# NoakLiu/FastFourierDiffusion

Measured on AMD Instinct MI355X. Metric: samples/sec at 1000 diffusion steps, ECG freq-domain, higher is better.
Workload: dtype f32; 1 GPU; ECG frequency-domain L=187 C=1, transformer d72/H12/NL10/F2048, VP beta[0.1,20], 1000-step sampler (BASELINE configs[1]); batch_per_gpu=512, global_batch=512, diffusion_steps=1000, cache=False, noise=philox on device

## Files before the change

### fastfourierdiffusion_amd/csrc/ffd_api.hip

```cpp
#include <math.h>
#include <stdarg.h>
#include <stdio.h>
#include <string.h>

#include <algorithm>
#include <string>
#include <vector>

#include "../../include/ffd.h"
#include "ffd_internal.h"

using namespace ffd;

namespace {

template <typename T>
struct Grow {
  T* p = nullptr;
  size_t cap = 0;
};

struct WeightSlot {
  std::string key;
  size_t n;
// ... 204 lines not shown
  if (g_ffn_split) {
    p.ffn = FFN_SPLIT;
  } else if (hp && g_ffn_height == 1) {
    p.ffn = FFN_LN_OPROJ, p.mb = hp;
  } else if (!(hp && g_small_wgs == 0) && (p.ns = small_path_splits(M, d, F))) {
    p.ffn = FFN_SMALL, p.part_floats = small_path_partial_floats(M, d, p.ns);
  } else if (pk.ring && !(hp && g_rows_slices == 0) && rows_slice_plan(M, d, F, &p.nw, &p.nslice, &unf)) {
    p.ffn = unf ? FFN_ROWS_SLICED : FFN_ROWS_SLICED_OPROJ, p.cps = 2, p.part_floats = rows_slice_floats(M, d, p.nslice);
  } else if ((p.nm = hp && g_mid_path == 1 ? 0 : mid_path_splits(M, d, F))) {
    p.ffn = FFN_MID, p.part_floats = small_path_partial_floats(cdiv(M, 64) * 64, d, p.nm);
  } else if (pk.ring && ffn_rows_fused_selected(M, d, F)) {
    p.ffn = FFN_ROWS_OPROJ, p.nw = rows_nw(), p.cps = 2;
  } else if (pk.ring && ffn_rows_selected(M, d, F)) {
    p.ffn = FFN_ROWS, p.nw = rows_nw(), p.cps = g_ffn_rows_cps == 1 && d == 72 ? 1 : 2;
  } else {
    p.ffn = FFN_LN;
    p.mb = g_ffn_mb_override >= 1 ? g_ffn_mb_override : cdiv(M, 64) >= 512 ? 4 : cdiv(M, 32) >= 512 ? 2 : 1;
    if (hp) p.mb = hp;
    p.persist = g_ffn_persist;
  }
  if (p.ffn == FFN_LN || p.ffn == FFN_LN_OPROJ) p.rem = g_ffn_rem && ffn_rem_rows(d, p.mb);
  p.oproj_separate = p.ffn >= FFN_ROWS_SLICED;
  p.swap = p.ffn == FFN_ROWS_SLICED_OPROJ || p.ffn == FFN_ROWS_OPROJ;
  return p;
}

LstmPlan plan_lstm(const ffd_model_desc& m, int B) {
  const int maxb = lstm_wave_max_batch(m.max_len, m.d_model);
  if (g_lstm_wave && m.d_model % 4 == 0 && m.d_model >= 16 && m.num_layers <= 64 && maxb >= 16)
    return {true, B < maxb ? B : maxb};
  return {false, B};
}

}

extern "C" {

int ffd_tune(const char* key, int value) {
  if (!key) return FFD_ERR_INVALID;
  if (!strcmp(key, "reset")) {
#define FFD_KNOB_RESET(k, var, def, ...) var = def;
    FFD_KNOBS(FFD_KNOB_RESET, FFD_KNOB_RESET)
#undef FFD_KNOB_RESET
    return FFD_OK;
  }
  const int v = value;
// ... 387 lines not shown
                                hipStream_t s, unsigned long long* stamp = nullptr) {
  const ffd_model_desc& m = ctx->desc;
  const int L = m.max_len, d = m.d_model, H = m.n_head, hd = d / H;
  float* out = ctx->attn.p;
  if (p.attn == ATTN_FUSED) {
    const float* pack = p.q_only == 2 ? w.aw_kvq
                        : p.hpw == 2  ? (p.q_only ? w.aw_q2 : w.aw_full2)
                                      : (p.q_only ? w.aw_q : w.aw_full);
    return launch_qkv_attention(AttnArgs{x, pack, kt, vt, kt_out, vt_out, out, B, L, n_own, stamp,
                                         p.attn_static && w.attn_bounded && kt == nullptr},
                                d, hd, p.hpw, p.q_only, p.kspl, p.qg, s);
  }
  if (stamp != nullptr) return hipErrorInvalidValue;
  const size_t M = (size_t)B * L;
  float *q = ctx->qkv.p, *k = q + M * d, *v = q + 2 * M * d;
  hipError_t e = launch_linear_hm(x, p.q_only ? w.q_wp : w.in_wp, w.in_b, q, k, v, (int)M, p.q_only ? 1 : 3, d, L, H, hd, s);
  if (e == hipSuccess) e = launch_attention(q, k, v, kt, vt, out, B, L, H, hd, n_own, p.qg, s);
  if (e == hipSuccess && kt_out)
    e = launch_kv_store(k, v, kt_out, vt_out, L, H, hd, n_own, s);
  return e;
}

static hipError_t run_ffn(const ffd_ctx* ctx, const LayerPlan& p, const LayerWeights& w, const float* attn, float* cur,
                          float* alt, int M, hipStream_t s, unsigned long long* stamp = nullptr) {
  const int d = ctx->desc.d_model, F = ctx->desc.dim_feedforward;
  float* P = ctx->ffn_part.p;
  const bool sliced = p.ffn == FFN_ROWS_SLICED_OPROJ || p.ffn == FFN_ROWS_SLICED;
  const bool fused = p.ffn == FFN_ROWS_SLICED_OPROJ || p.ffn == FFN_ROWS_OPROJ;
  float* const y = fused ? alt : cur;
  const RowsArgs rows{fused ? attn : alt, fused ? cur : nullptr, &w, sliced ? P : y, M, d, F, p.nw, p.cps, fused,
                      sliced ? p.nslice : 0, stamp};
  switch (p.ffn) {
    case FFN_LN_OPROJ:
      return stamp ? hipErrorInvalidValue : launch_oproj_ffn_ln(attn, cur, w, cur, M, d, F, p.mb, p.rem, s);
    case FFN_SMALL:
      return stamp ? hipErrorInvalidValue : launch_oproj_ffn_small(attn, cur, w, alt, P, cur, M, d, F, p.ns, s);
    case FFN_ROWS_SLICED_OPROJ:
    case FFN_ROWS_SLICED: {
      if (stamp || p.nslice < 2) return hipErrorInvalidValue;
      const hipError_t e = launch_ffn_rows(rows, s);
      return e != hipSuccess ? e : launch_rows_reduce_ln(P, w, y, M, d, p.nslice, s);
    }
    case FFN_ROWS_OPROJ:
    case FFN_ROWS: return launch_ffn_rows(rows, s);
    case FFN_MID:
      return stamp ? hipErrorInvalidValue : launch_ffn_mid(alt, w, P, cur, M, d, F, p.nm, s);
    case FFN_SPLIT: return launch_ffn_ln_split(alt, w, cur, M, d, F, s, stamp);
    case FFN_LN: return launch_ffn_ln(alt, w, cur, M, d, F, p.mb, p.rem, p.persist, s, stamp);
  }
  return hipErrorInvalidValue;
}

static const struct {
  const char* name;
  bool oproj;
} kFfnForms[] = {
    {"k_ffn_ln<oproj>", true},
    {"k_oproj_ffn_split + k_ffn_reduce_ln", true},
    {"k_ffn_rows<oproj, sliced> + k_rows_reduce_ln", true},
    {"k_ffn_rows<oproj>", true},
    {"k_ffn_rows<sliced> + k_rows_reduce_ln", false},
    {"k_ffn_part", false},
    {"k_ffn_ln_split", false},
    {"k_ffn_rows", false},
    {"k_ffn_ln", false},
};

static int forward_impl(ffd_ctx* ctx, const float* x, const float* temb, int temb_stride, float* score_out,
                        float* crf_out, int B, int n_rec, hipStream_t s, const float** hidden_out = nullptr) {
  const ffd_model_desc& m = ctx->desc;
  const int L = m.max_len, C = m.n_channels, d = m.d_model, M = B * L;
  const ModelWeights& mw = ctx->model;
  if (m.kind == FFD_MODEL_MLP) {
    const int io = L * C, F = m.dim_feedforward;
    HIPCHECK(launch_dense(x, mw.embed_w, mw.embed_b, temb_stride ? nullptr : temb, temb_stride ? temb : nullptr,
                          ctx->h0.p, B, d, io, 0, s));
    float* cur = ctx->h0.p;
    float* alt = ctx->h1.p;
    for (const MlpLayer& l : ctx->mlp) {
      HIPCHECK(launch_dense(cur, l.w0, l.b0, nullptr, nullptr, ctx->qkv.p, B, F, d, 1, s));
      HIPCHECK(launch_dense(ctx->qkv.p, l.w3, l.b3, nullptr, cur, alt, B, d, F, 0, s));
      std::swap(cur, alt);
    }
    HIPCHECK(launch_dense(cur, mw.unembed_w, mw.unembed_b, nullptr, nullptr, score_out, B, io, d, 0, s));
    return FFD_OK;
  }
  float* const h0 = ctx->h0.p;
  if (m.kind == FFD_MODEL_LSTM) {
    TIMED(FFD_K_EMBED, launch_embed(x, mw.embed_w, mw.embed_b, nullptr, temb, temb_stride, h0, B, L, C, d, s));
    if (const LstmPlan lp = plan_lstm(m, B); lp.wave) {
      const int Bw = lp.Bw;
      if (int rc = ensure(ctx, ctx->lstm_prog, (size_t)16 + 16 * cdiv(Bw, 16))) return rc;
      const float *wih[64], *whh[64], *bs[64];
      for (int i = 0; i < m.num_layers; ++i) wih[i] = ctx->lstm[i].ih_wpk, whh[i] = ctx->lstm[i].hh_wpk, bs[i] = ctx->lstm[i].b_wpk;
      if (int rc = ensure(ctx, ctx->lstm_state, lstm_wave_state_floats(Bw, d, m.num_layers))) return rc;
      for (int b0 = 0; b0 < B; b0 += Bw) {
        const int nb = B - b0 < Bw ? B - b0 : Bw;
        TIMED(FFD_K_LSTM_REC, launch_lstm_wave(h0 + (size_t)b0 * L * d, wih, whh, bs, m.num_layers, nb, L, d,
                                               ctx->lstm_prog.p, ctx->lstm_state.p, ctx->async_err, s,
                                               b0 == 0 ? ctx->lstm_trace : nullptr));
      }
    } else
    for (const LstmLayer& l : ctx->lstm) {
      if (int rc = ensure(ctx, ctx->qkv, (size_t)M * 4 * d)) return rc;
      TIMED(FFD_K_LSTM_GATES, launch_linear(h0, l.wih_p, l.bsum, ctx->qkv.p, M, 4 * d, d, 4 * d, s));
      TIMED(FFD_K_LSTM_REC, launch_lstm_layer(h0, ctx->qkv.p, l.whh, B, L, d, s));
    }
    if (hidden_out) {
      *hidden_out = h0;
      return FFD_OK;
    }
    TIMED(FFD_K_UNEMBED, launch_unembed(h0, mw.unembed_w, mw.unembed_b, score_out, M, C, d, s));
    return FFD_OK;
  }
  const int H = m.n_head, hd = d / H, F = m.dim_feedforward;
  TIMED(FFD_K_EMBED, launch_embed(x, mw.embed_w, mw.embed_b, mw.pos, temb, temb_stride, h0, B, L, C, d, s));
  const CacheMode mode = cache_mode(n_rec, L);
  const CacheUse cu = cache_use(mode, n_rec, L);
  const size_t lt = (size_t)H * L * hd;
  if (g_ffn_split && !ffn_split_supported(d, F))
    return ctx->fail(FFD_ERR_UNSUPPORTED, "ffn_split needs d_model %% 4 == 0, d_model <= 96, dim_feedforward %% 128 == 0");
  const LayerPlan plan = plan_of(ctx, B, mode);
  if (plan.attn == ATTN_TWO_KERNEL)
    if (int rc = ensure(ctx, ctx->qkv, (size_t)M * 3 * d)) return rc;
  if (int rc = ensure(ctx, ctx->ffn_part, plan.part_floats)) return rc;
  float* const attn = ctx->attn.p;
  float* cur = h0;
  float* alt = ctx->h1.p;
  for (int i = 0; i < m.num_layers; ++i) {
    LayerWeights& w = ctx->layers[i];
    float* kt = ctx->kt ? ctx->kt + i * lt : nullptr;
    float* vt = ctx->vt ? ctx->vt + i * lt : nullptr;
    TIMED(FFD_K_ATTN, run_attention(ctx, plan, w, cur, cu.tables ? kt : nullptr, cu.tables ? vt : nullptr,
                                    cu.store ? kt : nullptr, cu.store ? vt : nullptr, B, cu.n_own, s));
    if (plan.ffn == FFN_SPLIT && w.w1s == nullptr) {
      if (int rc = dev_alloc(ctx, &w.w1s, w1split_bytes(d, F) / sizeof(float))) return rc;
      if (int rc = dev_alloc(ctx, &w.w2s, w2split_bytes(d, F) / sizeof(float))) return rc;
      HIPCHECK(launch_pack_ffn_split(w.w1, w.w2, w.w1s, w.w2s, d, F, s));
    }
    if (plan.oproj_separate)
      TIMED(FFD_K_OUTPROJ, launch_linear_res_ln(attn, w.out_wp, w.out_b, cur, w.n1w, w.n1b, alt, M, d, s));
    TIMED(FFD_K_FFN, run_ffn(ctx, plan, w, attn, cur, alt, M, s));
    if (plan.swap) std::swap(cur, alt);
    if (mode == CACHE_FULL) {
      HIPCHECK(launch_linear_hm(cur, w.kv_wp, w.in_b + d, kt, vt, nullptr, L, 2, d, L, H, hd, s));
    }
    if (n_rec >= 0 && crf_out)
      HIPCHECK(hipMemcpyAsync(crf_out + (size_t)i * L * d, cur, sizeof(float) * L * d, hipMemcpyDeviceToDevice, s));
  }
  if (n_rec >= 0) {
    if (mode == CACHE_FULL) ctx->stats.recompute_count += (int64_t)L * m.num_layers, ctx->table_allocated = true;
    else if (mode == CACHE_PURE) ctx->stats.cache_hit_count += (int64_t)L * m.num_layers;
    else if (mode == CACHE_MIXED) {
      ctx->stats.cache_hit_count += (int64_t)(L - n_rec) * m.num_layers;
      ctx->stats.recompute_count += (int64_t)n_rec * m.num_layers;
      ctx->table_allocated = true;
    }
  }
  if (hidden_out) {
    *hidden_out = cur;
    return FFD_OK;
  }
  TIMED(FFD_K_UNEMBED, launch_unembed(cur, mw.unembed_w, mw.unembed_b, score_out, M, C, d, s));
  return FFD_OK;
}

static int check_async(ffd_ctx* ctx) {
  if (!ctx->async_err) return FFD_OK;
  const int code = *reinterpret_cast<volatile int*>(ctx->async_err);
  if (code == 0) return FFD_OK;
  *reinterpret_cast<volatile int*>(ctx->async_err) = 0;
  return ctx->fail(FFD_ERR_STATE,
                   "k_lstm_wave: unit %d waited longer than %d ms for the unit it depends on (the layer wavefront needs the "
                   "device's compute units to itself: another stream or process was holding some); the results of that "
                   "launch are invalid", code - 1, g_lstm_wave_spin_ms);
}

static int check_ready(ffd_ctx* ctx, int B) {
  if (int rc = check_async(ctx)) return rc;
  if (!ctx->finalized) return ctx->fail(FFD_ERR_STATE, "weights not finalised (call ffd_finalize_weights)");
// ... 190 lines not shown
  const ffd_model_desc& m = ctx->desc;
  const int d = m.d_model;
  hipStream_t s = (hipStream_t)stream;
  if (ctx->fresca_on) {
    if ((rc = ensure(ctx, ctx->score2, (size_t)B * m.max_len * m.n_channels))) return rc;
    if ((rc = ensure(ctx, ctx->fwork, (size_t)B * m.n_channels * (m.max_len / 2 + 1) + 4))) return rc;
  }
  if ((int)ctx->ts_host.size() != n_steps || memcmp(ctx->ts_host.data(), timesteps, sizeof(float) * n_steps) != 0 ||
      ctx->temb_epoch != ctx->weight_epoch) {
    HIPCHECK(hipStreamSynchronize(s));
    if ((rc = ensure(ctx, ctx->temb_tab, (size_t)n_steps * d))) return rc;
    if ((rc = ensure(ctx, ctx->ts_dev, (size_t)n_steps))) return rc;
    ctx->ts_host.assign(timesteps, timesteps + n_steps);
    HIPCHECK(hipMemcpy(ctx->ts_dev.p, ctx->ts_host.data(), sizeof(float) * n_steps, hipMemcpyHostToDevice));
    if ((rc = time_embed(ctx, ctx->ts_dev.p, 0.f, n_steps, ctx->temb_tab.p, s))) return rc;
    ctx->temb_epoch = ctx->weight_epoch;
  }
  const size_t slab = (size_t)B * m.max_len * m.n_channels;
  const uint64_t elem_off = sample_offset * (uint64_t)m.max_len * m.n_channels;
  const bool fuse_tail = tail_fusable(ctx) && (m.n_channels % 4 != 0 || elem_off % 4 == 0) &&
                         (m.n_channels % 4 != 0 || reinterpret_cast<uintptr_t>(x) % 16 == 0) &&
                         (!z_inject || m.n_channels % 4 != 0 ||
                          (reinterpret_cast<uintptr_t>(z_inject) % 16 == 0 && slab % 4 == 0));
  for (int j = 0; j < n_run; ++j) {
    const int i = first_step + j;
    int n_rec = -1;
    if (use_cache) {
      const int gstep = global_step0 + j;
      ctx->stats.current_step = gstep;
      n_rec = ffd_host_gate(gstep, m.max_len, ctx->ccfg.K, ctx->ccfg.R);
    }
    float* crf_dst = nullptr;
    float* crf_copy = nullptr;
    if (use_cache && ctx->crf_cap_on) {
      const ffd_crf_capture_cfg& cc = ctx->crf_cap;
      const int gstep = global_step0 + j;
      const size_t crf_n = (size_t)m.num_layers * m.max_len * d;
      if (cc.ring && gstep % cc.every == 0) crf_dst = cc.ring + (size_t)((gstep / cc.every) % cc.n_slots) * crf_n;
      if (cc.last && gstep % cc.last_every == 0) {
        const int rest = n_run - 1 - j;
        const int to_next = cc.last_every - (gstep % cc.last_every);
        if (to_next > rest) {
          if (crf_dst) crf_copy = cc.last; else crf_dst = cc.last;
        }
      }
    }
    const float* hidden = nullptr;
    if ((rc = forward_impl(ctx, x, ctx->temb_tab.p + (size_t)i * d, 0, ctx->score.p, crf_dst, B, n_rec, s,
// ... 339 lines not shown
```

### fastfourierdiffusion_amd/csrc/ffd_elem.hip

```cpp
#include <math.h>

#include <algorithm>

#include "ffd_internal.h"

namespace ffd {

__global__ void k_pack_dweight(const float* __restrict__ W, float* __restrict__ Wp, int N, int D) {
  const int G = dpack_groups(D);
  const size_t total = dpack_floats(N, D);
  for (size_t i = (size_t)blockIdx.x * blockDim.x + threadIdx.x; i < total; i += (size_t)gridDim.x * blockDim.x) {
    int j = i & 3;
    int lane = (i >> 2) & 63;
    size_t rest = i >> 8;
    int g = rest % G;
    int nt = rest / G;
    int n = 16 * nt + (lane & 15);
    int k = 4 * (4 * g + j) + (lane >> 4);
    Wp[i] = (n < N && k < D) ? W[(size_t)n * D + k] : 0.f;
  }
}

__global__ void k_pack_w2(const float* __restrict__ W2, float* __restrict__ W2p, int D, int F) {
  const int CT = cdiv(D, 16);
// ... 289 lines not shown
  const unsigned total = (unsigned)((size_t)B * L * D);
  unsigned blocks = (total + 255) / 256;
  if (blocks > 16384) blocks = 16384;
  if (blocks < 1) blocks = 1;
  hipLaunchKernelGGL(k_add_table, dim3(blocks), dim3(256), 0, s, x, rowtab, battab, out, total, L, D);
  return hipGetLastError();
}

__global__ void k_renorm_rows_once(float* __restrict__ W, int D, float max_norm) {
  float* w = W + (size_t)blockIdx.x * D;
  float ss = 0.f;
  for (int k = threadIdx.x; k < D; k += WAVE) ss += w[k] * w[k];
  for (int o = 32; o > 0; o >>= 1) ss += __shfl_xor(ss, o);
  const float norm = sqrtf(ss);
  if (norm > max_norm) {
    const float scale = max_norm / (norm + 1e-7f);
    for (int k = threadIdx.x; k < D; k += WAVE) w[k] *= scale;
  }
}

static hipError_t launch_renorm_rows_once(float* W, int rows, int D, float max_norm, hipStream_t s) {
  hipLaunchKernelGGL(k_renorm_rows_once, dim3(rows), dim3(WAVE), 0, s, W, D, max_norm);
  return hipGetLastError();
}

__device__ __forceinline__ float sde_update(float xi, float sc, float Gl, float zz, const SdeParams& p) {
  const float g = __fmul_rn(p.cs, Gl);
  const float g2 = __fmul_rn(g, g);
  const float gs = __fmul_rn(g2, sc);
  const float drift = (p.sde == 0) ? __fsub_rn(__fmul_rn(p.a, xi), gs) : -gs;
  const float t1 = __fsub_rn(xi, __fmul_rn(drift, p.dt));
  return __fadd_rn(t1, __fmul_rn(p.sqdt, __fmul_rn(g, zz)));
}

__global__ __launch_bounds__(256) void k_sde_step_v4(float* __restrict__ x, const float* __restrict__ score,
                                                     const float* __restrict__ z, const float* __restrict__ G,
                                                     SdeParams p, uint64_t seed, uint64_t elem_offset, uint32_t step,
                                                     size_t nvec, int L, unsigned C4) {
  for (size_t v = (size_t)blockIdx.x * blockDim.x + threadIdx.x; v < nvec; v += (size_t)gridDim.x * blockDim.x) {
    const float4 xi = reinterpret_cast<const float4*>(x)[v];
    const float4 sc = reinterpret_cast<const float4*>(score)[v];
    float zz[4];
    if (z) {
      const float4 zv = reinterpret_cast<const float4*>(z)[v];
      zz[0] = zv.x, zz[1] = zv.y, zz[2] = zv.z, zz[3] = zv.w;
    } else {
      normal4((elem_offset >> 2) + v, seed, step, zz);
    }
    const float Gl = G[(v / C4) % (size_t)L];
    reinterpret_cast<float4*>(x)[v] = float4{sde_update(xi.x, sc.x, Gl, zz[0], p), sde_update(xi.y, sc.y, Gl, zz[1], p),
                                             sde_update(xi.z, sc.z, Gl, zz[2], p), sde_update(xi.w, sc.w, Gl, zz[3], p)};
  }
}

__global__ void k_sde_step(float* __restrict__ x, const float* __restrict__ score, const float* __restrict__ z,
// ... 401 lines not shown
```

### fastfourierdiffusion_amd/csrc/ffd_ffn_rows.hip

```cpp
#include "ffd_internal.h"

namespace ffd {

typedef float f32x16 __attribute__((ext_vector_type(16)));
__device__ __forceinline__ f32x16 mfma32(float a, float b, f32x16 c) {
  return __builtin_amdgcn_mfma_f32_32x32x2f32(a, b, c, 0, 0, 0);
}

constexpr __host__ __device__ int ring_ct(int D) { return D / 32; }
constexpr __host__ __device__ int ring_ng(int D) { return (D % 32) / 4; }
constexpr __host__ __device__ int ring_ks2(int D) { return 16 * ring_ct(D) + 4 * ((ring_ng(D) + 1) / 2); }
constexpr __host__ __device__ int ring_nq1(int D) { return cdiv(ring_ks2(D), 4); }
constexpr __host__ __device__ int ring_kperm(int D, int s, int half) {
  return s < 16 * ring_ct(D) ? 32 * (s / 16) + 8 * ((s % 16) / 4) + 4 * half + s % 4
                             : 32 * ring_ct(D) + 4 * (2 * ((s - 16 * ring_ct(D)) / 4) + half) + (s - 16 * ring_ct(D)) % 4;
}
constexpr __host__ __device__ int ring_nmain(int D) { return ring_nq1(D) + 4 * ring_ct(D); }
constexpr __host__ __device__ int ring_nrem(int D) { return 4 * ring_ng(D); }
constexpr __host__ __device__ int ring_nfc(int D) { return ring_nmain(D) + ring_nrem(D); }
constexpr __host__ __device__ bool ring_compact(int D) { return D != 72; }
constexpr __host__ __device__ int ring_nfull(int D) { return ring_compact(D) ? ring_nmain(D) : ring_nfc(D); }
constexpr __host__ __device__ int ring_chunk_groups(int D) { return ring_nfull(D) + cdiv(ring_nfc(D) - ring_nfull(D), 8) + 1; }
constexpr __host__ __device__ int ring_frag_off(int nmain, int k, int lane) {
  return k < nmain ? k * 256 + lane * 4
// ... 210 lines not shown
#pragma unroll
  for (int i = 0; i < (NG + 1) / 2; ++i) {
    float a[4];
#pragma unroll
    for (int e = 0; e < 4; ++e) {
      float t0 = rem[2 * i][e];
      t0 += __shfl_xor(t0, 32);
      float t1 = 0.f;
      if (2 * i + 1 < NG) {
        t1 = rem[(2 * i + 1 < NG) ? 2 * i + 1 : 0][e];
        t1 += __shfl_xor(t1, 32);
      }
      a[e] = half ? t1 : t0;
    }
    vr[i] = float4{a[0], a[1], a[2], a[3]};
    if (first && 2 * i + half < NG) {
      const float4 bq = *reinterpret_cast<const float4*>(&p[32 * CT + 4 * (2 * i + half)]);
      const float4 x4 = resrem[i];
      vr[i] = float4{x4.x + (a[0] + bq.x), x4.y + (a[1] + bq.y), x4.z + (a[2] + bq.z), x4.w + (a[3] + bq.w)};
    }
  }
}

template <int D, int NW, int CPS, int NSLOT, int PR, bool OP, bool SL, bool ONE>
__global__ __launch_bounds__(64 * NW, 3) void k_ffn_rows(const float* __restrict__ X, const float* __restrict__ Rin,
                                                             const float* __restrict__ ring, const float* __restrict__ ringp,
                                                             const float* __restrict__ b2, const float* __restrict__ gam,
                                                             const float* __restrict__ bet, const float* __restrict__ bo,
                                                             const float* __restrict__ gam1, const float* __restrict__ bet1,
                                                             float* __restrict__ Y, int M, int F, int nslice,
                                                             unsigned long long* stamp) {
  using C = FfnRowsCfg<D, NW, CPS, NSLOT>;
  constexpr int KS2 = C::KS2, CT = C::CT, NG = C::NG, NQ1 = C::NQ1, SGC = C::SGC, NFC = C::NFC, PD = C::PD;
  constexpr int NGA = NG > 0 ? NG : 1, CTA = CT > 0 ? CT : 1;
  constexpr int NRH = (NG + 1) / 2;
  constexpr int NRA = NRH > 0 ? NRH : 1;
  constexpr int R = 32 * NW;
  constexpr int NFS = CPS * NFC;
  constexpr int RPG = cdiv(4, CTA);
  constexpr int NPM = C::NPM, NFP = C::NFP;
  static_assert(CT == 0 || 4 % CT == 0, "relu placement assumes CT in {1, 2, 4}");
  static_assert(!OP || (CPS == 2 && C::AHEAD == 2 && NFP + PD <= NFS + PD && C::NFPP <= C::SLOT_G && CT > 0),
                "the fused form: two-chunk slots, ring one slot ahead of the barrier");
  __shared__ __align__(16) float lds[C::LDS_FLOATS];

  const int lane = threadIdx.x & 63;
  const int wave = __builtin_amdgcn_readfirstlane(threadIdx.x >> 6);
  const int half = lane >> 5, m = lane & 31;
  float* const ringl = lds;
  float* const lnp = lds + NSLOT * C::SLOT_FLOATS;
  const unsigned ring_base = __builtin_amdgcn_readfirstlane(lds_addr(ringl));

  const int ntiles = (M + R - 1) / R;
  const int slice = SL ? (int)blockIdx.x % nslice : 0;
  const int slot_first = SL ? slice * (F / (32 * CPS)) / nslice : 0;
  const int nchunk_slots = SL ? (slice + 1) * (F / (32 * CPS)) / nslice - slot_first : F / (32 * CPS);
  const int NSL = nchunk_slots + (OP ? 1 : 0);
  const int tstride = SL ? (int)gridDim.x / nslice : (int)gridDim.x;
  const int my_tiles = SL ? ((int)blockIdx.x / nslice < ntiles ? (ntiles - 1 - (int)blockIdx.x / nslice) / tstride + 1 : 0)
                       : ONE ? ((int)blockIdx.x < ntiles ? 1 : 0)
                             : ((int)blockIdx.x < ntiles) ? (ntiles - 1 - (int)blockIdx.x) / (int)gridDim.x + 1 : 0;
  const int total = my_tiles * NSL;
  if (total == 0) return;

  const float* const ring_s = ring + (size_t)slot_first * C::SLOT_FLOATS;
  auto slot_src = [&](int wslot) -> const float* {
    return OP ? (wslot == 0 ? ringp : ring_s + (size_t)(wslot - 1) * C::SLOT_FLOATS) : ring_s + (size_t)wslot * C::SLOT_FLOATS;
// ... 22 lines not shown
    for (int ct = 0; ct < CT; ++ct)
#pragma unroll
      for (int t = 0; t < 4; ++t) asm volatile("" : "+v"(q[ct][t].x), "+v"(q[ct][t].y), "+v"(q[ct][t].z), "+v"(q[ct][t].w));
#pragma unroll
    for (int i = 0; i < NRH; ++i) asm volatile("" : "+v"(qrem[i].x), "+v"(qrem[i].y), "+v"(qrem[i].z), "+v"(qrem[i].w));
  };
  auto xb_of = [&](int s) -> float {
    return s < 16 * CT ? f4e(xv[s / 16 < CTA ? s / 16 : 0][(s % 16) / 4], s % 4)
                       : f4e(xrem[(s - 16 * CT) / 4 < NRH ? (s - 16 * CT) / 4 : 0], (s - 16 * CT) % 4);
  };
  auto zero_acc = [&]() {
#pragma unroll
    for (int ct = 0; ct < CTA; ++ct)
#pragma unroll
      for (int r = 0; r < 16; ++r) yacc[ct][r] = 0.f;
#pragma unroll
    for (int g = 0; g < NGA; ++g) yrem[g] = f32x4{0.f, 0.f, 0.f, 0.f};
  };

  static_assert(C::AHEAD == 2 || !OP, "prologue of the fused form");
  for (int i = threadIdx.x; i < (OP ? 6 : 3) * D; i += 64 * NW)
    lnp[i] = i < D ? b2[i] : i < 2 * D ? gam[i - D] : i < 3 * D ? bet[i - 2 * D]
           : i < 4 * D ? bo[i - 3 * D] : i < 5 * D ? gam1[i - 4 * D] : bet1[i - 5 * D];
  {
    const float* src = slot_src(0);
    for (int g = wave; g < (OP ? C::NFPP : C::SLOT_G); g += NW) dma_piece_sbase(src + g * 256, lane * 16, ring_base + g * 1024);
  }
  float4 rin[CTA][4], rinrem[NRA];
  load_rows(X, xv, xrem);
  if (OP) load_rows(Rin, rin, rinrem);
  wait_vm<0>();
  retire_rows(xv, xrem);
  if (OP) retire_rows(rin, rinrem);
#pragma unroll
  for (int j = 1; j < C::AHEAD; ++j)
    if (j < total) {
      const float* src = slot_src(j % NSL);
      const unsigned dst = ring_base + (unsigned)(j % NSLOT) * (C::SLOT_FLOATS * 4);
#pragma unroll
      for (int i = 0; i < C::NPW; ++i) {
        const int g0 = wave + i * NW, g = g0 < C::SLOT_G ? g0 : g0 - C::SLOT_G;
        dma_piece_sbase(src + g * 256, lane * 16, dst + g * 1024);
      }
    }
  asm volatile("s_waitcnt lgkmcnt(0)" ::: "memory");
  __builtin_amdgcn_s_barrier();
// ... 167 lines not shown
            } else {
              wait_vm<0>();
            }
            __builtin_amdgcn_s_barrier();
          }
          __builtin_amdgcn_sched_barrier(0);
        }
      }
#pragma unroll
      for (int k = 0; k < PD; ++k) f[k] = f[NFS + k];
      if (dma_on && ++wnext == NSL) wnext = 0;
    }

    if (stamp) {
      const unsigned long long rt = __builtin_amdgcn_s_memrealtime();
      st_acc += __builtin_amdgcn_s_memtime() - st_clk;
      st_acc_rt += rt - st_rt;
      if (st_tiles == 0) st_first_e = rt;
    }
    {
      float4 v[CTA][4], vr[NRA];
      if (SL) raw_rows<D>(yacc, yrem, xv, xrem, lnp, half, slice == 0, v, vr);
      else ln_rows<D>(yacc, yrem, xv, xrem, lnp, half, v, vr);
      const int row = tile * R + wave * 32 + m;
      if (row < M) {
        float* yr = Y + ((size_t)(SL ? slice : 0) * M + row) * D;
#pragma unroll
        for (int ct = 0; ct < CT; ++ct)
#pragma unroll
          for (int t = 0; t < 4; ++t) *reinterpret_cast<float4*>(yr + 32 * ct + 8 * t + 4 * half) = v[ct][t];
#pragma unroll
        for (int i = 0; i < (NG + 1) / 2; ++i)
          if (2 * i + half < NG) *reinterpret_cast<float4*>(yr + 32 * CT + 4 * (2 * i + half)) = vr[i];
      }
    }
    if (stamp) {
      if (st_tiles == 0) st_epi = __builtin_amdgcn_s_memrealtime();
      ++st_tiles;
    }
    tile += tstride;
    if (tl + 1 < my_tiles) {
      load_rows(X, xv, xrem);
      if (OP) load_rows(Rin, rin, rinrem);
      retire_rows(xv, xrem);
      if (OP) retire_rows(rin, rinrem);
    }
  }
#undef FFD_SLOT_PRELUDE
// ... 94 lines not shown
  *nw_out = bnw, *nslice_out = bs, *unfused_out = bunf;
  return true;
}
size_t rows_slice_floats(int M, int D, int nslice) { return (size_t)nslice * M * D; }

int rows_waves(int M) {
  const double eff[3] = {0.85, 0.915, 0.938};
  double best = 0.0;
  int nw = 0;
  for (int i = 2; i >= 0; --i) {
    const int cand = 4 * (i + 1);
    const double t = (double)cdiv(cdiv(M, 32 * cand), num_cus()) * (i + 1) / eff[i];
    if (best == 0.0 || t < best * 0.999) best = t, nw = cand;
  }
  return nw;
}

#endif

template <int D, int NW, int CPS, int NSLOT>
static hipError_t launch_rows_cfg(const RowsArgs& a, hipStream_t s) {
  const int R = 32 * NW;
  const int ntiles = cdiv(a.M, R);
  constexpr int per_cu_lds = (160 * 1024) / (FfnRowsCfg<D, NW, CPS, NSLOT>::LDS_FLOATS * 4);
  constexpr int per_cu = per_cu_lds < 12 / NW ? per_cu_lds : 12 / NW;
  const int slots = per_cu * num_cus();
  const int gsl = a.nslice > 0 ? (slots / a.nslice < ntiles ? slots / a.nslice : ntiles) : 0;
  const int grid = a.nslice > 0 ? gsl * a.nslice : ntiles < slots ? ntiles : slots;
  const LayerWeights& w = *a.w;
  constexpr int PRV = NW > 4 ? 1 : 0;
#define FFD_ROWS_LAUNCH2(PR, OP, SL, ONE)                                                                              \
  hipLaunchKernelGGL((k_ffn_rows<D, NW, CPS, NSLOT, PR, OP, SL, ONE>), dim3(grid), dim3(64 * NW), 0, s, a.X, a.Rin,     \
                     w.ring, w.ring_op, w.b2, w.n2w, w.n2b, w.out_b, w.n1w, w.n1b, a.Y, a.M, a.F, a.nslice, a.stamp)
#define FFD_ROWS_LAUNCH(PR, OP, SL)                                                                                    \
  do {                                                                                                                 \
    if constexpr (!(SL)) {                                                                                             \
      if (grid == ntiles) FFD_ROWS_LAUNCH2(PR, OP, false, true); else FFD_ROWS_LAUNCH2(PR, OP, false, false);          \
    } else {                                                                                                           \
      FFD_ROWS_LAUNCH2(PR, OP, true, false);                                                                           \
    }                                                                                                                  \
  } while (0)
  if constexpr (CPS == 2 && NSLOT == 3) {
    if (a.fused) {
      if constexpr (NW >= 8) {
        if (a.nslice > 0) {
          if (gsl < 1 || a.nslice > a.F / 64) return hipErrorInvalidValue;
          FFD_ROWS_LAUNCH(PRV, true, true);
          return hipGetLastError();
        }
      }
      if (a.nslice > 0) return hipErrorInvalidValue;
      FFD_ROWS_LAUNCH(PRV, true, false);
      return hipGetLastError();
    }
  }
  if (a.fused) return hipErrorInvalidValue;
  if (a.nslice > 0) {
    if constexpr (CPS == 2 && NSLOT == 3 && NW >= 8) {
      if (gsl < 1 || a.nslice > a.F / 64) return hipErrorInvalidValue;
      FFD_ROWS_LAUNCH(PRV, false, true);
      return hipGetLastError();
    }
// ... 59 lines not shown
```

### fastfourierdiffusion_amd/csrc/ffd_internal.h

```cpp
#pragma once
#include <hip/hip_runtime.h>
#include <stdint.h>

#include "../../include/ffd.h"

namespace ffd {

constexpr int WAVE = 64;

#define FFD_D_LIST(X) X(8) X(16) X(24) X(32) X(48) X(60) X(64) X(72)
#define FFD_HD_LIST(X) X(2) X(3) X(4) X(5) X(6) X(8)

typedef float f32x4 __attribute__((ext_vector_type(4)));

__device__ __forceinline__ f32x4 mfma16(float a, float b, f32x4 c) {
  return __builtin_amdgcn_mfma_f32_16x16x4f32(a, b, c, 0, 0, 0);
}

constexpr __host__ __device__ int cdiv(int a, int b) { return (a + b - 1) / b; }

__device__ __forceinline__ float relu_bits(float x) {
  const int i = __builtin_bit_cast(int, x);
  return __builtin_bit_cast(float, i > 0 ? i : 0);
}
// ... 68 lines not shown
  I("ffn_rows_nw", g_ffn_rows_nw, 0, v == 0 || v == 4 || v == 8 || v == 12)   \
  I("ffn_rows_cps", g_ffn_rows_cps, 0, v >= 0 && v <= 2)   \
  B("ffn_rows_fuse", g_ffn_rows_fuse, 1)                   \
  I("rows_slices", g_rows_slices, 0, v >= -1 && v != 1 && v <= 32)   \
  I("rows_slices_fuse", g_rows_slices_fuse, 0, v >= 0 && v <= 2)   \
  I("mid_path", g_mid_path, 1, v == 0 || v == 1 || v == 2 || v == 4 || v == 8)   \
  B("small_path", g_small_path, 1)                         \
  I("small_wgs", g_small_wgs, 0, v >= 0)                   \
  I("attn_small", g_attn_small, 1, v == 0 || v == 1 || v == 2 || v == 4)   \
  I("attn_fused", g_attn_fused, 1, v >= 0 && v <= 1)       \
  I("attn_hpw", g_attn_hpw, 0, v >= 0 && v <= 2)           \
  I("attn_qg", g_attn_qg, 0, v >= 0 && v <= 3)             \
  B("attn_kvq", g_attn_kvq, 1)                             \
  B("attn_static_bound", g_attn_static_bound, 1)           \
  B("embed_ldsx", g_embed_ldsx, 1)                         \
  I("embed_threads", g_embed_threads, 262144, v >= 256)    \
  I("lstm_wave", g_lstm_wave, 1, v >= 0 && v <= 2)         \
  B("lstm_wave_persist", g_lstm_wave_persist, 1)           \
  I("lstm_wave_per", g_lstm_wave_per, 0, v >= 0 && v <= 16)   \
  I("lstm_wave_chunk", g_lstm_wave_chunk, 0, v >= 0 && !(v > 1 && (v & 1)) && v <= 1024)   \
  I("lstm_wave_fault", g_lstm_wave_fault, 0, v >= 0)       \
  I("lstm_wave_spin_ms", g_lstm_wave_spin_ms, 2000, v >= 1 && v <= 20000)   \
  B("fuse_tail", g_fuse_tail, 1)                           \
  I("fail_alloc_after", g_fail_alloc_after, 0, v >= 0)

#define FFD_KNOB_DECL(key, var, ...) extern thread_local int var;
FFD_KNOBS(FFD_KNOB_DECL, FFD_KNOB_DECL)
#undef FFD_KNOB_DECL

template <int N>
__device__ __forceinline__ void wait_vm() {
  asm volatile("s_waitcnt vmcnt(%0)" ::"n"(N) : "memory");
}

__device__ __forceinline__ void dma_piece(const float* g, unsigned lds_byte) {
  asm volatile("s_mov_b32 m0, %0\n\ts_nop 0\n\tglobal_load_lds_dwordx4 %1, off" ::"s"(lds_byte), "v"(g)
               : "memory");
}
__device__ __forceinline__ void dma_piece_sbase(const float* base, unsigned lane_byte, unsigned lds_byte) {
  asm volatile("s_mov_b32 m0, %0\n\ts_nop 0\n\tglobal_load_lds_dwordx4 %1, %2" ::"s"(lds_byte), "v"(lane_byte), "s"(base)
               : "memory");
}
__device__ __forceinline__ unsigned lds_addr(const float* p) {
  return (unsigned)(unsigned long)((const __attribute__((address_space(3))) float*)p);
}

// ... 24 lines not shown
};

hipError_t launch_pack_dweight(const float* W, float* Wp, int N, int D, hipStream_t s);
hipError_t launch_pack_w2(const float* W2, float* W2p, int D, int F, hipStream_t s);
constexpr __host__ __device__ int w2rem_groups(int D) { return (D % 16) / 4; }
constexpr __host__ __device__ size_t w2rem_floats(int D, int F) { return (size_t)(F / 16) * (w2rem_groups(D) ? w2rem_groups(D) : 1) * 64 * 4; }
hipError_t launch_pack_w2rem(const float* W2, float* W2r, int D, int F, hipStream_t s);
hipError_t launch_renorm_rows(float* W, int rows, int D, float max_norm, hipStream_t s);

hipError_t launch_time_embed(const float* ts, float t_imm, int n, const float* W, const float* dense_w,
                             const float* dense_b, float* temb, int D, hipStream_t s);
hipError_t launch_embed(const float* X, const float* We, const float* be, const float* pos, const float* temb,
                        int temb_stride, float* h, int B, int L, int C, int D, hipStream_t s);
hipError_t launch_unembed(const float* h, const float* Wu, const float* bu, float* score, int M, int C, int D,
                          hipStream_t s);

struct SdeParams {
  int sde;
  float a;
  float cs;
  float dt, sqdt;
};
SdeParams sde_params(int sde, double a, double b, double t, float step_size);
hipError_t launch_sde_step(float* x, const float* score, const float* z, const float* G, SdeParams p, uint64_t seed,
                           uint64_t elem_offset, uint32_t step, int B, int L, int C, hipStream_t s);
bool unembed_sde_supported(int C, int D);
hipError_t launch_unembed_sde(const float* h, const float* Wu, const float* bu, float* x, const float* z, const float* G,
                              SdeParams p, uint64_t seed, uint64_t elem_offset, uint32_t step, int B, int L, int C,
                              int D, hipStream_t s);

constexpr uint32_t SM_TAG_NOISE = 0xFFFFFFFEu, SM_TAG_TIMES = 0xFFFFFFFDu;
hipError_t launch_sm_perturb(const float* x0, float* x_noisy, const float* mean_coeff, const float* sigma, const float* G,
                             const float* z, uint64_t seed, uint64_t sample_offset, int B, int L, int C, hipStream_t s);
hipError_t launch_sm_loss(const float* score, const float* sigma, const float* G, const float* z, uint64_t seed,
                          uint64_t sample_offset, int likelihood_weighting, int reduce_mean, double* out, int B, int L,
                          int C, hipStream_t s);

hipError_t launch_linear(const float* X, const float* Wp, const float* bias, float* Y, int M, int N, int D, int ldy,
                         hipStream_t s);
hipError_t launch_linear_res_ln(const float* X, const float* Wp, const float* bias, const float* R, const float* g,
                                const float* beta, float* Y, int M, int D, hipStream_t s);
bool ffn_rem_rows(int D, int mb);
hipError_t launch_ffn_ln(const float* X, const LayerWeights& w, float* Y, int M, int D, int F, int mb, bool rem, int persist,
                         hipStream_t s, unsigned long long* stamp = nullptr);
int ffn_height_plan(int M, int D, int F);
hipError_t launch_oproj_ffn_ln(const float* attn, const float* Rres, const LayerWeights& w, float* Y, int M, int D, int F,
                               int mb, bool rem, hipStream_t s);
bool ffn_rows_supported(int D, int F);
bool ffn_rows_selected(int M, int D, int F);
size_t ffn_ring_floats(int D, int F);
hipError_t launch_pack_ffn_ring(const float* W1, const float* b1, const float* W2, float* out, int D, int F, hipStream_t s);
struct RowsArgs {
  const float *X, *Rin;
  const LayerWeights* w;
  float* Y;
  int M, D, F;
  int nw, cps;
  bool fused;
  int nslice;
  unsigned long long* stamp;
};
int rows_waves(int M);
hipError_t launch_ffn_rows(const RowsArgs& a, hipStream_t s);
bool ffn_rows_fused_selected(int M, int D, int F);
size_t ffn_ring_oproj_floats(int D);
hipError_t launch_pack_oproj_ring(const float* Wo, float* out, int D, hipStream_t s);
bool rows_slice_plan(int M, int D, int F, int* nw_out, int* nslice_out, int* unfused_out);
size_t rows_slice_floats(int M, int D, int nslice);
hipError_t launch_rows_reduce_ln(const float* P, const LayerWeights& w, float* Y, int M, int D, int nslice, hipStream_t s);
int small_path_splits(int M, int D, int F);
size_t small_path_partial_floats(int M, int D, int NS);
hipError_t launch_oproj_ffn_small(const float* attn, const float* xres, const LayerWeights& w, float* x1, float* P,
                                  float* Y, int M, int D, int F, int NS, hipStream_t s);
int mid_path_splits(int M, int D, int F);
hipError_t launch_ffn_mid(const float* x1, const LayerWeights& w, float* P, float* Y, int M, int D, int F, int NS, hipStream_t s);
bool ffn_split_supported(int D, int F);
size_t w1split_bytes(int D, int F);
size_t w2split_bytes(int D, int F);
hipError_t launch_pack_ffn_split(const float* W1, const float* W2, void* w1s, void* w2s, int D, int F, hipStream_t s);
hipError_t launch_ffn_ln_split(const float* X, const LayerWeights& w, float* Y, int M, int D, int F, hipStream_t s,
                               unsigned long long* stamp = nullptr);
constexpr float ATTN_SCORE_T = 64.0f;
float attn_q_scale(int hd);
// ... 63 lines not shown
               FFN_LN };
struct PackSet {
  bool aw_full, aw_full2, aw_kvq;
  bool ring;
};
struct LayerPlan {
  AttnForm attn;
  int hpw;
  int q_only;
  int kspl;
  int qg;
  bool attn_static;
  FfnForm ffn;
  int mb;
  bool rem;
  int persist;
  int ns;
  int nw, cps;
  int nslice;
  int nm;
  bool oproj_separate;
  bool swap;
  size_t part_floats;
};
LayerPlan plan_layer(const ffd_model_desc& m, int B, CacheMode mode, const PackSet& packs);
struct LstmPlan {
  bool wave;
  int Bw;
};
LstmPlan plan_lstm(const ffd_model_desc& m, int B);

}
```

Measured before the change: 100.5 samples/s.

## Fuse unembed, SDE step and next-step embed into last-layer FFN rows kernel

For single-channel transformer sampling, the last layer's k_ffn_rows kernel now computes the unembed dot product per row, applies the SDE update with on-device normals, writes x, and writes the next step's embedding directly into the hidden buffer. This removes the separate unembed/SDE kernel and the embed kernel from each diffusion step, along with their launches and the round trips of the hidden state through global memory. In exchange the kernel needs extra LDS for the tail constants, which can lower occupancy per CU, and the sampler loop gains a separate code path.

```diff
diff --git a/fastfourierdiffusion_amd/csrc/ffd_api.hip b/fastfourierdiffusion_amd/csrc/ffd_api.hip
--- a/fastfourierdiffusion_amd/csrc/ffd_api.hip
+++ b/fastfourierdiffusion_amd/csrc/ffd_api.hip
@@ -250,6 +250,8 @@
   if (p.ffn == FFN_LN || p.ffn == FFN_LN_OPROJ) p.rem = g_ffn_rem && ffn_rem_rows(d, p.mb);
   p.oproj_separate = p.ffn >= FFN_ROWS_SLICED;
   p.swap = p.ffn == FFN_ROWS_SLICED_OPROJ || p.ffn == FFN_ROWS_OPROJ;
+  p.tail_in_ffn = g_tail_in_ffn && g_fuse_tail && m.n_channels == 1 &&
+                  (p.ffn == FFN_ROWS_OPROJ || (p.ffn == FFN_ROWS && p.cps == 2));
   return p;
 }
 
@@ -683,14 +685,16 @@
 }
 
 static hipError_t run_ffn(const ffd_ctx* ctx, const LayerPlan& p, const LayerWeights& w, const float* attn, float* cur,
-                          float* alt, int M, hipStream_t s, unsigned long long* stamp = nullptr) {
+                          float* alt, int M, hipStream_t s, unsigned long long* stamp = nullptr,
+                          const TailArgs* tail = nullptr) {
   const int d = ctx->desc.d_model, F = ctx->desc.dim_feedforward;
   float* P = ctx->ffn_part.p;
   const bool sliced = p.ffn == FFN_ROWS_SLICED_OPROJ || p.ffn == FFN_ROWS_SLICED;
   const bool fused = p.ffn == FFN_ROWS_SLICED_OPROJ || p.ffn == FFN_ROWS_OPROJ;
   float* const y = fused ? alt : cur;
   const RowsArgs rows{fused ? attn : alt, fused ? cur : nullptr, &w, sliced ? P : y, M, d, F, p.nw, p.cps, fused,
-                      sliced ? p.nslice : 0, stamp};
+                      sliced ? p.nslice : 0, stamp, tail};
+  if (tail && !p.tail_in_ffn) return hipErrorInvalidValue;
   switch (p.ffn) {
     case FFN_LN_OPROJ:
       return stamp ? hipErrorInvalidValue : launch_oproj_ffn_ln(attn, cur, w, cur, M, d, F, p.mb, p.rem, s);
@@ -727,8 +731,14 @@
     {"k_ffn_ln", false},
 };
 
+struct StepTail {
+  const TailArgs* tail;
+  bool embed;
+  float* start;
+};
 static int forward_impl(ffd_ctx* ctx, const float* x, const float* temb, int temb_stride, float* score_out,
-                        float* crf_out, int B, int n_rec, hipStream_t s, const float** hidden_out = nullptr) {
+                        float* crf_out, int B, int n_rec, hipStream_t s, const float** hidden_out = nullptr,
+                        StepTail* st = nullptr) {
   const ffd_model_desc& m = ctx->desc;
   const int L = m.max_len, C = m.n_channels, d = m.d_model, M = B * L;
   const ModelWeights& mw = ctx->model;
@@ -775,19 +785,21 @@
     return FFD_OK;
   }
   const int H = m.n_head, hd = d / H, F = m.dim_feedforward;
-  TIMED(FFD_K_EMBED, launch_embed(x, mw.embed_w, mw.embed_b, mw.pos, temb, temb_stride, h0, B, L, C, d, s));
+  float* cur = st ? st->start : h0;
+  float* alt = cur == h0 ? ctx->h1.p : h0;
+  if (!st || st->embed)
+    TIMED(FFD_K_EMBED, launch_embed(x, mw.embed_w, mw.embed_b, mw.pos, temb, temb_stride, cur, B, L, C, d, s));
   const CacheMode mode = cache_mode(n_rec, L);
   const CacheUse cu = cache_use(mode, n_rec, L);
   const size_t lt = (size_t)H * L * hd;
   if (g_ffn_split && !ffn_split_supported(d, F))
     return ctx->fail(FFD_ERR_UNSUPPORTED, "ffn_split needs d_model %% 4 == 0, d_model <= 96, dim_feedforward %% 128 == 0");
   const LayerPlan plan = plan_of(ctx, B, mode);
+  if (st && (!plan.tail_in_ffn || n_rec >= 0)) return ctx->fail(FFD_ERR_STATE, "step tail without a plan for it");
   if (plan.attn == ATTN_TWO_KERNEL)
     if (int rc = ensure(ctx, ctx->qkv, (size_t)M * 3 * d)) return rc;
   if (int rc = ensure(ctx, ctx->ffn_part, plan.part_floats)) return rc;
   float* const attn = ctx->attn.p;
-  float* cur = h0;
-  float* alt = ctx->h1.p;
   for (int i = 0; i < m.num_layers; ++i) {
     LayerWeights& w = ctx->layers[i];
     float* kt = ctx->kt ? ctx->kt + i * lt : nullptr;
@@ -801,7 +813,7 @@
     }
     if (plan.oproj_separate)
       TIMED(FFD_K_OUTPROJ, launch_linear_res_ln(attn, w.out_wp, w.out_b, cur, w.n1w, w.n1b, alt, M, d, s));
-    TIMED(FFD_K_FFN, run_ffn(ctx, plan, w, attn, cur, alt, M, s));
+    TIMED(FFD_K_FFN, run_ffn(ctx, plan, w, attn, cur, alt, M, s, nullptr, st && i == m.num_layers - 1 ? st->tail : nullptr));
     if (plan.swap) std::swap(cur, alt);
     if (mode == CACHE_FULL) {
       HIPCHECK(launch_linear_hm(cur, w.kv_wp, w.in_b + d, kt, vt, nullptr, L, 2, d, L, H, hd, s));
@@ -817,6 +829,10 @@
       ctx->stats.recompute_count += (int64_t)n_rec * m.num_layers;
       ctx->table_allocated = true;
     }
+  }
+  if (st) {
+    st->start = cur;
+    return FFD_OK;
   }
   if (hidden_out) {
     *hidden_out = cur;
@@ -1053,8 +1069,21 @@
                          (m.n_channels % 4 != 0 || reinterpret_cast<uintptr_t>(x) % 16 == 0) &&
                          (!z_inject || m.n_channels % 4 != 0 ||
                           (reinterpret_cast<uintptr_t>(z_inject) % 16 == 0 && slab % 4 == 0));
+  const bool tail_in_ffn = fuse_tail && !use_cache && m.kind == FFD_MODEL_TRANSFORMER && m.num_layers >= 1 &&
+                           ctx->model.pos != nullptr && plan_of(ctx, B, CACHE_STD).tail_in_ffn;
+  StepTail st{nullptr, true, ctx->h0.p};
   for (int j = 0; j < n_run; ++j) {
     const int i = first_step + j;
+    if (tail_in_ffn) {
+      const ModelWeights& mw = ctx->model;
+      const TailArgs ta{mw.unembed_w, mw.unembed_b, x, z_inject ? z_inject + (size_t)j * slab : nullptr, ctx->G_dev,
+                        sde_params(m.sde, m.sde_a, m.sde_b, (double)timesteps[i], step_size), seed, elem_off, (uint32_t)i,
+                        m.max_len, mw.embed_w, mw.embed_b, mw.pos,
+                        j + 1 < n_run ? ctx->temb_tab.p + (size_t)(i + 1) * d : nullptr};
+      st.tail = &ta, st.embed = j == 0;
+      if ((rc = forward_impl(ctx, x, ctx->temb_tab.p + (size_t)i * d, 0, nullptr, nullptr, B, -1, s, nullptr, &st))) return rc;
+      continue;
+    }
     int n_rec = -1;
     if (use_cache) {
       const int gstep = global_step0 + j;
diff --git a/fastfourierdiffusion_amd/csrc/ffd_elem.hip b/fastfourierdiffusion_amd/csrc/ffd_elem.hip
--- a/fastfourierdiffusion_amd/csrc/ffd_elem.hip
+++ b/fastfourierdiffusion_amd/csrc/ffd_elem.hip
@@ -335,15 +335,6 @@
 static hipError_t launch_renorm_rows_once(float* W, int rows, int D, float max_norm, hipStream_t s) {
   hipLaunchKernelGGL(k_renorm_rows_once, dim3(rows), dim3(WAVE), 0, s, W, D, max_norm);
   return hipGetLastError();
-}
-
-__device__ __forceinline__ float sde_update(float xi, float sc, float Gl, float zz, const SdeParams& p) {
-  const float g = __fmul_rn(p.cs, Gl);
-  const float g2 = __fmul_rn(g, g);
-  const float gs = __fmul_rn(g2, sc);
-  const float drift = (p.sde == 0) ? __fsub_rn(__fmul_rn(p.a, xi), gs) : -gs;
-  const float t1 = __fsub_rn(xi, __fmul_rn(drift, p.dt));
-  return __fadd_rn(t1, __fmul_rn(p.sqdt, __fmul_rn(g, zz)));
 }
 
 __global__ __launch_bounds__(256) void k_sde_step_v4(float* __restrict__ x, const float* __restrict__ score,
diff --git a/fastfourierdiffusion_amd/csrc/ffd_ffn_rows.hip b/fastfourierdiffusion_amd/csrc/ffd_ffn_rows.hip
--- a/fastfourierdiffusion_amd/csrc/ffd_ffn_rows.hip
+++ b/fastfourierdiffusion_amd/csrc/ffd_ffn_rows.hip
@@ -256,14 +256,23 @@
   }
 }
 
-template <int D, int NW, int CPS, int NSLOT, int PR, bool OP, bool SL, bool ONE>
+template <bool TAIL>
+struct TailParam {};
+template <>
+struct TailParam<true> {
+  TailArgs a;
+};
+template <int D>
+constexpr int tail_lds_floats() { return cdiv(4 * D + 1, 4) * 4; }
+
+template <int D, int NW, int CPS, int NSLOT, int PR, bool OP, bool SL, bool TAIL, bool ONE>
 __global__ __launch_bounds__(64 * NW, 3) void k_ffn_rows(const float* __restrict__ X, const float* __restrict__ Rin,
                                                              const float* __restrict__ ring, const float* __restrict__ ringp,
                                                              const float* __restrict__ b2, const float* __restrict__ gam,
                                                              const float* __restrict__ bet, const float* __restrict__ bo,
                                                              const float* __restrict__ gam1, const float* __restrict__ bet1,
                                                              float* __restrict__ Y, int M, int F, int nslice,
-                                                             unsigned long long* stamp) {
+                                                             unsigned long long* stamp, TailParam<TAIL> tp) {
   using C = FfnRowsCfg<D, NW, CPS, NSLOT>;
   constexpr int KS2 = C::KS2, CT = C::CT, NG = C::NG, NQ1 = C::NQ1, SGC = C::SGC, NFC = C::NFC, PD = C::PD;
   constexpr int NGA = NG > 0 ? NG : 1, CTA = CT > 0 ? CT : 1;
@@ -276,7 +285,9 @@
   static_assert(CT == 0 || 4 % CT == 0, "relu placement assumes CT in {1, 2, 4}");
   static_assert(!OP || (CPS == 2 && C::AHEAD == 2 && NFP + PD <= NFS + PD && C::NFPP <= C::SLOT_G && CT > 0),
                 "the fused form: two-chunk slots, ring one slot ahead of the barrier");
-  __shared__ __align__(16) float lds[C::LDS_FLOATS];
+  static_assert(!TAIL || (!SL && CPS == 2), "the tail: whole rows, two-chunk slots");
+  static_assert((C::LDS_FLOATS + (TAIL ? tail_lds_floats<D>() : 0)) * 4 <= 160 * 1024, "LDS");
+  __shared__ __align__(16) float lds[C::LDS_FLOATS + (TAIL ? tail_lds_floats<D>() : 0)];
 
   const int lane = threadIdx.x & 63;
   const int wave = __builtin_amdgcn_readfirstlane(threadIdx.x >> 6);
@@ -345,6 +356,13 @@
   for (int i = threadIdx.x; i < (OP ? 6 : 3) * D; i += 64 * NW)
     lnp[i] = i < D ? b2[i] : i < 2 * D ? gam[i - D] : i < 3 * D ? bet[i - 2 * D]
            : i < 4 * D ? bo[i - 3 * D] : i < 5 * D ? gam1[i - 4 * D] : bet1[i - 5 * D];
+  if constexpr (TAIL) {
+    const TailArgs& ta = tp.a;
+    float* const tl = lnp + C::LNP_PAD;
+    for (int i = threadIdx.x; i < 4 * D + 1; i += 64 * NW)
+      tl[i] = i < D ? ta.We[i] : i < 2 * D ? ta.be[i - D] : i < 3 * D ? (ta.temb_next ? ta.temb_next[i - 2 * D] : 0.f)
+            : i < 4 * D ? ta.Wu[i - 3 * D] : ta.bu[0];
+  }
   {
     const float* src = slot_src(0);
     for (int g = wave; g < (OP ? C::NFPP : C::SLOT_G); g += NW) dma_piece_sbase(src + g * 256, lane * 16, ring_base + g * 1024);
@@ -558,8 +576,69 @@
       float4 v[CTA][4], vr[NRA];
       if (SL) raw_rows<D>(yacc, yrem, xv, xrem, lnp, half, slice == 0, v, vr);
       else ln_rows<D>(yacc, yrem, xv, xrem, lnp, half, v, vr);
-      const int row = tile * R + wave * 32 + m;
-      if (row < M) {
+      if constexpr (TAIL) {
+        const TailArgs& ta = tp.a;
+        const float* const tl = lnp + C::LNP_PAD;
+        int lane_t;
+        asm volatile("v_mbcnt_lo_u32_b32 %0, -1, 0\n\tv_mbcnt_hi_u32_b32 %0, -1, %0" : "=v"(lane_t));
+        const int half = lane_t >> 5;
+        const int row = tile * R + wave * 32 + (lane_t & 31);
+        float sc = tl[4 * D];
+#pragma unroll
+        for (int g = 0; g < cdiv(D, 16); ++g) {
+          float4 own[2], oth[2];
+#pragma unroll
+          for (int jj = 0; jj < 2; ++jj) {
+            const int j = 2 * g + jj;
+            own[jj] = j < 4 * CT ? v[j / 4 < CTA ? j / 4 : 0][j % 4]
+                    : j - 4 * CT < NRH ? vr[j - 4 * CT < NRH ? j - 4 * CT : 0] : float4{0.f, 0.f, 0.f, 0.f};
+            oth[jj] = float4{0.f, 0.f, 0.f, 0.f};
+            if (8 * j < D)
+              oth[jj] = float4{__shfl_xor(own[jj].x, 32), __shfl_xor(own[jj].y, 32), __shfl_xor(own[jj].z, 32),
+                               __shfl_xor(own[jj].w, 32)};
+          }
+#pragma unroll
+          for (int e = 0; e < 4; ++e)
+#pragma unroll
+            for (int q = 0; q < 4; ++q) {
+              const int k = 16 * g + 4 * q + e;
+              if (k < D) {
+                const float a = f4e(own[q >> 1], e), b = f4e(oth[q >> 1], e);
+                sc = fmaf(tl[3 * D + k], (q & 1) == half ? a : b, sc);
+              }
+            }
+          asm volatile("" : "+v"(sc));
+          __builtin_amdgcn_sched_barrier(0);
+        }
+        if (row < M) {
+          const int l = row % ta.L;
+          const float xi = ta.x[row];
+          float zz[4];
+          load_normals(ta.z, (size_t)row, 1, ta.seed, ta.elem_offset, ta.step, zz);
+          const float xn = sde_update(xi, sc, ta.G[l], zz[0], ta.p);
+          if (half == 0) ta.x[row] = xn;
+          if (ta.temb_next) {
+            const float* pr = ta.pos + (size_t)l * D;
+            float* yr = Y + (size_t)row * D;
+            auto emb = [&](int c0) {
+              const float4 w4 = *reinterpret_cast<const float4*>(&tl[c0]);
+              const float4 b4 = *reinterpret_cast<const float4*>(&tl[D + c0]);
+              const float4 t4 = *reinterpret_cast<const float4*>(&tl[2 * D + c0]);
+              const float4 p4 = *reinterpret_cast<const float4*>(pr + c0);
+              *reinterpret_cast<float4*>(yr + c0) =
+                  float4{(fmaf(xn, w4.x, b4.x) + p4.x) + t4.x, (fmaf(xn, w4.y, b4.y) + p4.y) + t4.y,
+                         (fmaf(xn, w4.z, b4.z) + p4.z) + t4.z, (fmaf(xn, w4.w, b4.w) + p4.w) + t4.w};
+            };
+#pragma unroll
+            for (int ct = 0; ct < CT; ++ct)
+#pragma unroll
+              for (int t = 0; t < 4; ++t) emb(32 * ct + 8 * t + 4 * half);
+#pragma unroll
+            for (int i = 0; i < (NG + 1) / 2; ++i)
+              if (2 * i + half < NG) emb(32 * CT + 4 * (2 * i + half));
+          }
+        }
+      } else if (const int row = tile * R + wave * 32 + m; row < M) {
         float* yr = Y + ((size_t)(SL ? slice : 0) * M + row) * D;
 #pragma unroll
         for (int ct = 0; ct < CT; ++ct)
@@ -700,22 +779,34 @@
 static hipError_t launch_rows_cfg(const RowsArgs& a, hipStream_t s) {
   const int R = 32 * NW;
   const int ntiles = cdiv(a.M, R);
-  constexpr int per_cu_lds = (160 * 1024) / (FfnRowsCfg<D, NW, CPS, NSLOT>::LDS_FLOATS * 4);
+  constexpr int per_cu_lds = (160 * 1024) / ((FfnRowsCfg<D, NW, CPS, NSLOT>::LDS_FLOATS + tail_lds_floats<D>()) * 4);
   constexpr int per_cu = per_cu_lds < 12 / NW ? per_cu_lds : 12 / NW;
   const int slots = per_cu * num_cus();
   const int gsl = a.nslice > 0 ? (slots / a.nslice < ntiles ? slots / a.nslice : ntiles) : 0;
   const int grid = a.nslice > 0 ? gsl * a.nslice : ntiles < slots ? ntiles : slots;
   const LayerWeights& w = *a.w;
   constexpr int PRV = NW > 4 ? 1 : 0;
-#define FFD_ROWS_LAUNCH2(PR, OP, SL, ONE)                                                                              \
-  hipLaunchKernelGGL((k_ffn_rows<D, NW, CPS, NSLOT, PR, OP, SL, ONE>), dim3(grid), dim3(64 * NW), 0, s, a.X, a.Rin,     \
-                     w.ring, w.ring_op, w.b2, w.n2w, w.n2b, w.out_b, w.n1w, w.n1b, a.Y, a.M, a.F, a.nslice, a.stamp)
+#define FFD_ROWS_LAUNCH2(PR, OP, SL, ONE, TL, tailp)                                                                   \
+  hipLaunchKernelGGL((k_ffn_rows<D, NW, CPS, NSLOT, PR, OP, SL, TL, ONE>), dim3(grid), dim3(64 * NW), 0, s, a.X, a.Rin, \
+                     w.ring, w.ring_op, w.b2, w.n2w, w.n2b, w.out_b, w.n1w, w.n1b, a.Y, a.M, a.F, a.nslice, a.stamp,    \
+                     tailp)
 #define FFD_ROWS_LAUNCH(PR, OP, SL)                                                                                    \
   do {                                                                                                                 \
+    if constexpr (!(SL) && CPS == 2) {                                                                                 \
+      if (a.tail) {                                                                                                    \
+        if (a.stamp) return hipErrorInvalidValue;                                                                      \
+        const TailParam<true> tpv{*a.tail};                                                                            \
+        if (grid == ntiles) FFD_ROWS_LAUNCH2(PR, OP, false, true, true, tpv);                                          \
+        else FFD_ROWS_LAUNCH2(PR, OP, false, false, true, tpv);                                                        \
+        break;                                                                                                         \
+      }                                                                                                                \
+    }                                                                                                                  \
+    if (a.tail) return hipErrorInvalidValue;                                                                           \
     if constexpr (!(SL)) {                                                                                             \
-      if (grid == ntiles) FFD_ROWS_LAUNCH2(PR, OP, false, true); else FFD_ROWS_LAUNCH2(PR, OP, false, false);          \
+      if (grid == ntiles) FFD_ROWS_LAUNCH2(PR, OP, false, true, false, TailParam<false>{});                            \
+      else FFD_ROWS_LAUNCH2(PR, OP, false, false, false, TailParam<false>{});                                          \
     } else {                                                                                                           \
-      FFD_ROWS_LAUNCH2(PR, OP, true, false);                                                                           \
+      FFD_ROWS_LAUNCH2(PR, OP, true, false, false, TailParam<false>{});                                                \
     }                                                                                                                  \
   } while (0)
   if constexpr (CPS == 2 && NSLOT == 3) {
diff --git a/fastfourierdiffusion_amd/csrc/ffd_internal.h b/fastfourierdiffusion_amd/csrc/ffd_internal.h
--- a/fastfourierdiffusion_amd/csrc/ffd_internal.h
+++ b/fastfourierdiffusion_amd/csrc/ffd_internal.h
@@ -114,6 +114,7 @@
   I("lstm_wave_fault", g_lstm_wave_fault, 0, v >= 0)       \
   I("lstm_wave_spin_ms", g_lstm_wave_spin_ms, 2000, v >= 1 && v <= 20000)   \
   B("fuse_tail", g_fuse_tail, 1)                           \
+  B("tail_in_ffn", g_tail_in_ffn, 1)                       \
   I("fail_alloc_after", g_fail_alloc_after, 0, v >= 0)
 
 #define FFD_KNOB_DECL(key, var, ...) extern thread_local int var;
@@ -184,6 +185,14 @@
   float dt, sqdt;
 };
 SdeParams sde_params(int sde, double a, double b, double t, float step_size);
+__device__ __forceinline__ float sde_update(float xi, float sc, float Gl, float zz, const SdeParams& p) {
+  const float g = __fmul_rn(p.cs, Gl);
+  const float g2 = __fmul_rn(g, g);
+  const float gs = __fmul_rn(g2, sc);
+  const float drift = (p.sde == 0) ? __fsub_rn(__fmul_rn(p.a, xi), gs) : -gs;
+  const float t1 = __fsub_rn(xi, __fmul_rn(drift, p.dt));
+  return __fadd_rn(t1, __fmul_rn(p.sqdt, __fmul_rn(g, zz)));
+}
 hipError_t launch_sde_step(float* x, const float* score, const float* z, const float* G, SdeParams p, uint64_t seed,
                            uint64_t elem_offset, uint32_t step, int B, int L, int C, hipStream_t s);
 bool unembed_sde_supported(int C, int D);
@@ -212,6 +221,17 @@
 bool ffn_rows_selected(int M, int D, int F);
 size_t ffn_ring_floats(int D, int F);
 hipError_t launch_pack_ffn_ring(const float* W1, const float* b1, const float* W2, float* out, int D, int F, hipStream_t s);
+struct TailArgs {
+  const float *Wu, *bu;
+  float* x;
+  const float *z, *G;
+  SdeParams p;
+  uint64_t seed, elem_offset;
+  uint32_t step;
+  int L;
+  const float *We, *be, *pos;
+  const float* temb_next;
+};
 struct RowsArgs {
   const float *X, *Rin;
   const LayerWeights* w;
@@ -221,6 +241,7 @@
   bool fused;
   int nslice;
   unsigned long long* stamp;
+  const TailArgs* tail = nullptr;
 };
 int rows_waves(int M);
 hipError_t launch_ffn_rows(const RowsArgs& a, hipStream_t s);
@@ -330,6 +351,7 @@
   bool oproj_separate;
   bool swap;
   size_t part_floats;
+  bool tail_in_ffn;
 };
 LayerPlan plan_layer(const ffd_model_desc& m, int B, CacheMode mode, const PackSet& packs);
 struct LstmPlan {
```

After: 101.0 samples/s (median of 6 runs). No clear change (+0.5%).
